# wahn/rs_pbrt

Hardware: NVIDIA H100
Metric: Mrays/s (higher is better)
Workload: dtype f32

## Files before the change

rs_pbrt_b200/csrc/pb_kernels.cuh:

```cuda
#pragma once
#include "pb_bsdf.cuh"
#include "pb_interaction.cuh"
#include "pb_sobol.cuh"
#include "pb_texture.cuh"
#include "pb_material.cuh"

namespace pb {

#define PB_TRACE_THREADS 128
#define PB_TRACE_SMEM_BYTES 49152
#define PB_SHADE_THREADS 128
#define PB_SMEM_SOBOL_BYTES 49152

#ifdef PB_HOST_EMU
PB_D void mbar_init(uint64_t*, uint32_t) {}
PB_D void mbar_fence_init() {}
PB_D void mbar_expect_tx(uint64_t*, uint32_t) {}
PB_D void tma_bulk_g2s(void* dst_smem, const void* src_gmem, uint32_t bytes, uint64_t*) { memcpy(dst_smem, src_gmem, bytes); }
PB_D void mbar_wait(uint64_t*, uint32_t) { __syncthreads(); }
#define PB_DYNAMIC_SMEM(name) unsigned char* name = emu::g_dyn_smem
#else
#define PB_DYNAMIC_SMEM(name) extern __shared__ __align__(16) unsigned char name[]
PB_D void mbar_fence_init() { asm volatile("fence.mbarrier_init.release.cluster;" ::: "memory"); }
PB_D uint32_t smem_u32(const void* p) { return (uint32_t)__cvta_generic_to_shared(p); }
// ... 288 lines not shown
            const float* p0 = vp + 3 * (size_t)(m.vbase + v0);
            const float* p1 = vp + 3 * (size_t)(m.vbase + v1);
            const float* p2 = vp + 3 * (size_t)(m.vbase + v2);
            tv[3 * (size_t)i] = make_float4(p0[0], p0[1], p0[2], p1[0]);
            tv[3 * (size_t)i + 1] = make_float4(p1[1], p1[2], p2[0], p2[1]);
            tv[3 * (size_t)i + 2] = make_float4(p2[2], __uint_as_float(material), __uint_as_float((uint32_t)area_light), __uint_as_float(m.flags));
            tidx[i] = make_uint4(m.vbase + v0, m.vbase + v1, m.vbase + v2, mesh);
        }
    }
    if (err) atomicMax(status, err);
}

__global__ void __launch_bounds__(256) k_wide_build(const float4* __restrict__ nodes, uint32_t n_nodes, float4* __restrict__ wide) {
    const uint32_t i = blockIdx.x * blockDim.x + threadIdx.x;
    if (i >= n_nodes) return;
    const float4 m1 = nodes[2 * (size_t)i + 1];
    const uint32_t meta = __float_as_uint(m1.w);
    if (meta & 0xffffu) return;
    const uint32_t c[2] = {i + 1u, __float_as_uint(m1.z)};
    float4 a[2], b[2];
    uint32_t ref[2];
    for (int k = 0; k < 2; ++k) {
        a[k] = nodes[2 * (size_t)c[k]];
        b[k] = nodes[2 * (size_t)c[k] + 1];
        const uint32_t cm = __float_as_uint(b[k].w), np = cm & 0xffffu;
        ref[k] = np ? (__float_as_uint(b[k].z) | (np << PB_WIDE_LEAF_SHIFT)) : c[k];
    }
    float4* o = wide + 4 * (size_t)i;
    o[0] = make_float4(a[0].x, a[0].y, a[0].z, a[0].w);
    o[1] = make_float4(b[0].x, b[0].y, a[1].x, a[1].y);
    o[2] = make_float4(a[1].z, a[1].w, b[1].x, b[1].y);
    o[3] = make_float4(__uint_as_float(ref[0]), __uint_as_float(ref[1]), __uint_as_float((meta >> 16) & 3u), 0.0f);
}
#ifndef PB_WIDE_MIN_BLOCKS
#define PB_WIDE_MIN_BLOCKS 0
#endif
#ifndef PB_WIDE_INST_MIN_BLOCKS
#define PB_WIDE_INST_MIN_BLOCKS 8
#endif
#if PB_WIDE_MIN_BLOCKS > 0
#define PB_WIDE_BOUNDS __launch_bounds__(PB_TRACE_THREADS, PB_WIDE_MIN_BLOCKS)
#else
#define PB_WIDE_BOUNDS __launch_bounds__(PB_TRACE_THREADS)
#endif
__global__ void PB_WIDE_BOUNDS k_trace_wide_plain(DScene sc, TraceIO io, const uint32_t* __restrict__ d_nrays, uint32_t* __restrict__ cursor, DCounters* cnt, int walk_steps) {
    trace_rays_wide<false>(sc, sc.wide, sc.tri_verts, io, *d_nrays, cursor, cnt, walk_steps);
}
__global__ void __launch_bounds__(PB_TRACE_THREADS, PB_WIDE_INST_MIN_BLOCKS) k_trace_wide_inst(DScene sc, TraceIO io, const uint32_t* __restrict__ d_nrays, uint32_t* __restrict__ cursor,
                                                                                             DCounters* cnt, int walk_steps) {
    trace_rays_wide<true>(sc, sc.wide, sc.tri_verts, io, *d_nrays, cursor, cnt, walk_steps);
}

__global__ void PB_WIDE_BOUNDS k_trace_wide_spec(DScene sc, TraceIO io, const uint32_t* __restrict__ d_nrays,
                                                                                        uint32_t* __restrict__ cursor, DCounters* cnt, int walk_steps) {
    trace_rays_wide_spec(sc, sc.wide, sc.tri_verts, io, *d_nrays, cursor, cnt, walk_steps);
}

__global__ void __launch_bounds__(256) k_rayprep(const float4* __restrict__ rays, const uint32_t* __restrict__ d_nrays, float4* __restrict__ pre) {
    const uint32_t n = *d_nrays;
    for (uint32_t i = blockIdx.x * blockDim.x + threadIdx.x; i < n; i += gridDim.x * blockDim.x) {
        const float4 a = rays[2 * (size_t)i], b = rays[2 * (size_t)i + 1];
        const RayPre r = make_ray(mk3(a.x, a.y, a.z), mk3(b.x, b.y, b.z));
        float4 p0, p1;
        pack_ray(r, p0, p1);
        pre[2 * (size_t)i] = p0;
        pre[2 * (size_t)i + 1] = p1;
    }
}

__global__ void __launch_bounds__(256) k_sort(DScene sc, DPaths ps, DLightGrid grid, uint32_t spatial, uint32_t instancing, const uint32_t* __restrict__ queue,
                                             const uint32_t* __restrict__ d_count, uint32_t* __restrict__ cls_queue, uint32_t cls_stride,
                                             uint32_t* __restrict__ cls_count, uint32_t* __restrict__ reset_count_out, uint32_t* __restrict__ reset_nrays) {
    if (blockIdx.x == 0 && threadIdx.x == 0) { *reset_count_out = 0u; *reset_nrays = 0u; }
    const uint32_t count = *d_count;
    const uint32_t lane = threadIdx.x & 31;
    const uint32_t total = (count + 31u) & ~31u;
    for (uint32_t qi = blockIdx.x * blockDim.x + threadIdx.x; qi < total; qi += gridDim.x * blockDim.x) {
        uint32_t cls = 0xffffffffu, slot = 0;
        if (qi < count) {
// ... 754 lines not shown
```

rs_pbrt_b200/csrc/pb_scene.cuh:

```cuda
#pragma once
#include "pb_math.cuh"

namespace pb {

enum LobeKind { LOBE_SPEC_REFL = 0, LOBE_SPEC_TRANS, LOBE_FRESNEL_SPEC, LOBE_LAMBERT, LOBE_OREN_NAYAR, LOBE_MF_REFL, LOBE_MF_TRANS, LOBE_FRESNEL_BLEND,
                LOBE_LAMBERT_TRANS  };
enum { BSDF_REFLECTION = 1, BSDF_TRANSMISSION = 2, BSDF_DIFFUSE = 4, BSDF_GLOSSY = 8, BSDF_SPECULAR = 16, BSDF_ALL = 31 };
enum FresnelKind { FRESNEL_NOOP = 0, FRESNEL_CONDUCTOR, FRESNEL_DIELECTRIC };

struct DLobe {
    int kind, type, fresnel;
    int has_sc;
    float r[3];
    float t[3];
    float eta_a, eta_b;
    float fr_a[3];
    float fr_k[3];
    float alpha_x, alpha_y;
    float on_a, on_b;
};
PB_HD float* lobe_sc_slot(DLobe& l) {
    if (l.kind == LOBE_FRESNEL_SPEC || l.kind == LOBE_FRESNEL_BLEND) return l.fr_k;
    return (l.kind == LOBE_SPEC_TRANS || l.kind == LOBE_LAMBERT_TRANS || l.kind == LOBE_MF_TRANS) ? l.r : l.t;
}
// ... 44 lines not shown
    float max_anisotropy;
    float su, sv, du, dv;
    uint32_t off[PB_MAX_MIP_LEVELS];
    uint32_t mapping;
    float map_m[16];
    uint32_t kind;
    float value[3];
    uint32_t child[3];
};
struct DMatSrc {
    uint32_t kind;
    float params[24];
    uint32_t tex[8];
    float alpha_u, alpha_v;
    uint8_t tex_off[8];
    uint32_t n_spectrum;
    uint32_t bump;
};
#define PB_MAT_BUMPED 0x200
#define PB_MAT_TEXTURED 0x100

enum { TRI_FLIP = 1, TRI_HAS_N = 2, TRI_HAS_UV = 4, TRI_HAS_S = 8, TRI_INSTANCE = 16 ,
       TRI_ALPHA = 32, TRI_SHADOW_ALPHA = 64  };

struct DInstance {
    uint32_t root, identity, pad0, pad1;
    float m[16], m_inv[16];
};

struct DScene {
    const float4* nodes;
    uint32_t n_nodes;
    const float4* wide;
    const float4* tri_verts;
    uint32_t n_tris;
    const uint4* tri_idx;
    const float* vn;
    const float* vuv;
    const float* vs;
    const DMaterial* materials;
    uint32_t n_materials;
    const DLight* lights;
    float world_radius;
    uint32_t n_lights;
    const DEnv* envs;
    const DInstance* instances;
    uint32_t n_instances;
    const uint2* mesh_alpha;
    const DTexture* textures;
    const DMatSrc* mat_src;
    const float* ewa_lut;
    uint32_t n_textures;
    float dx_camera[3], dy_camera[3];
    uint32_t n_inf;
    uint32_t inf[4];
    float raster_to_camera[16], camera_to_world[16];
    float lens_radius, focal_distance, shutter_open, shutter_close;
    float wb_min[3], wb_max[3];
};

struct DLightGrid {
    int nv[3];
    int n_lights;
    int* state;
    float* func;
    float* cdf;
// ... 79 lines not shown
```

rs_pbrt_b200/csrc/pb_trace.cuh:

```cuda
#pragma once
#include "pb_scene.cuh"

namespace pb {

struct RayPre {
    V3 o, d;
    V3 inv_dir;
    int neg[3];
    uint32_t negmask;
    int kx, ky, kz;
    float sx, sy, sz;
};

PB_D RayPre make_ray(V3 o, V3 d) {
    RayPre r;
    r.o = o;
    r.d = d;
    r.inv_dir = mk3(1.0f / d.x, 1.0f / d.y, 1.0f / d.z);
    r.neg[0] = r.inv_dir.x < 0.0f;
    r.neg[1] = r.inv_dir.y < 0.0f;
    r.neg[2] = r.inv_dir.z < 0.0f;
    r.negmask = (uint32_t)r.neg[0] | ((uint32_t)r.neg[1] << 1) | ((uint32_t)r.neg[2] << 2);
    r.kz = maxdim(abs3(d));
    r.kx = r.kz + 1; if (r.kx == 3) r.kx = 0;
// ... 115 lines not shown
PB_D void load_tri(const float4* __restrict__ tv, uint32_t i, V3& p0, V3& p1, V3& p2) {
    float4 a = __ldg(tv + 3 * (size_t)i), b = __ldg(tv + 3 * (size_t)i + 1), c = __ldg(tv + 3 * (size_t)i + 2);
    p0 = mk3(a.x, a.y, a.z);
    p1 = mk3(a.w, b.x, b.y);
    p2 = mk3(b.z, b.w, c.x);
}

struct WorkCount { uint32_t nodes, tris; };

#ifndef PB_SMEM_STACK_ENTRIES
#define PB_SMEM_STACK_ENTRIES 24
#endif
#define PB_TRACE_THREADS_ 128
#ifndef PB_LEAF_MIN
#define PB_LEAF_MIN 1
#endif
#ifndef PB_FLAT_WALK
#define PB_FLAT_WALK 1
#endif
#ifndef PB_REFILL_MIN
#define PB_REFILL_MIN 1
#endif
#ifndef PB_WALK_STEPS
#define PB_WALK_STEPS 16
#endif

#ifndef PB_CACHE_HINTS
#define PB_CACHE_HINTS 1
#endif
PB_D float4 ldg4_keep(const float4* p) {
#if PB_CACHE_HINTS
    float4 v;
    asm volatile("ld.global.nc.L1::evict_last.v4.f32 {%0,%1,%2,%3}, [%4];" : "=f"(v.x), "=f"(v.y), "=f"(v.z), "=f"(v.w) : "l"(p));
    return v;
#else
    return __ldg(p);
#endif
}
PB_D float4 ldg4_stream(const float4* p) {
#if PB_CACHE_HINTS
    float4 v;
    asm volatile("ld.global.nc.L1::no_allocate.v4.f32 {%0,%1,%2,%3}, [%4];" : "=f"(v.x), "=f"(v.y), "=f"(v.z), "=f"(v.w) : "l"(p));
    return v;
#else
    return __ldg(p);
#endif
}
PB_D float4 lds4(const float4* p) {
#ifdef PB_HOST_EMU
    return *p;
#else
    float4 v;
    asm volatile("ld.shared.v4.f32 {%0,%1,%2,%3}, [%4];" : "=f"(v.x), "=f"(v.y), "=f"(v.z), "=f"(v.w) : "r"((uint32_t)__cvta_generic_to_shared(p)));
    return v;
#endif
}

PB_D void xf_ray_dev(const float* __restrict__ m, V3 o, V3 d, float& t_max, V3& o_out, V3& d_out) {
    const float x = o.x, y = o.y, z = o.z;
    V3 ow = mk3(m[0] * x + m[1] * y + m[2] * z + m[3], m[4] * x + m[5] * y + m[6] * z + m[7], m[8] * x + m[9] * y + m[10] * z + m[11]);
    const float wp = m[12] * x + m[13] * y + m[14] * z + m[15];
    const V3 o_err = mk3(fabsf(m[0] * x) + fabsf(m[1] * y) + fabsf(m[2] * z) + fabsf(m[3]), fabsf(m[4] * x) + fabsf(m[5] * y) + fabsf(m[6] * z) + fabsf(m[7]),
                         fabsf(m[8] * x) + fabsf(m[9] * y) + fabsf(m[10] * z) + fabsf(m[11])) * gamma_n(3);
    if (wp != 1.0f) { const float inv = 1.0f / wp; ow = mk3(inv * ow.x, inv * ow.y, inv * ow.z); }
    const V3 dw = mk3(m[0] * d.x + m[1] * d.y + m[2] * d.z, m[4] * d.x + m[5] * d.y + m[6] * d.z, m[8] * d.x + m[9] * d.y + m[10] * d.z);
    const float ls = len2(dw);
// ... 444 lines not shown
            }
            if (!entered) {
                leaf_n = 0;
                if (!done) {
                    uint32_t nxt = 0;
                    PB_WPOP();
                    PB_WGOTO();
                }
            }
        }
        if (active && done) {
            if (INST && !any_hit && !hit_flag) best_prim = -1;
            const uint32_t slot = dest & PB_RAY_SLOT_MASK, kind = dest >> 30;
            if (kind == RAY_SHADOW) io.occl[slot] = best_prim >= 0 ? 1u : 0u;
            else {
                const float4 rec = make_float4(__int_as_float(best_prim), best.b0, best.b1, best.b2);
                if (kind == RAY_EXTEND) { io.hit[slot] = rec; if (INST) io.hit_inst[slot] = (uint32_t)best_inst; }
                else { io.mis_hit[slot] = rec; if (INST) io.mis_inst[slot] = (uint32_t)best_inst; }
            }
            active = false;
        }
    }
#undef PB_WPOP
#undef PB_WGOTO
#undef PB_WPUSH
    uint32_t a = n_closest, b = n_shadow;
    for (int o = 16; o > 0; o >>= 1) { a += __shfl_xor_sync(FULL, a, o); b += __shfl_xor_sync(FULL, b, o); }
    if (lane == 0) {
        if (a) atomicAdd(&cnt->closest_rays, (unsigned long long)a);
        if (b) atomicAdd(&cnt->shadow_rays, (unsigned long long)b);
    }
}

PB_D void trace_rays_wide_spec(const DScene& sc, const float4* __restrict__ wide, const float4* __restrict__ tris, const TraceIO& io, uint32_t n_rays,
                               uint32_t* __restrict__ cursor, DCounters* cnt, int walk_steps) {
    const unsigned FULL = 0xffffffffu;
    const int lane = threadIdx.x & 31;
    constexpr int NS = PB_WIDE_STACK_ENTRIES;
    __shared__ uint32_t s_ref[NS][PB_TRACE_THREADS_];
    __shared__ float s_tmin[NS][PB_TRACE_THREADS_];
    uint32_t l_ref[64 - NS];
    float l_tmin[64 - NS];
    RayPre r;
    float t_max = 0.0f, cur_tmin = 0.0f, leaf2_tmin = 0.0f;
    THit best;
    int best_prim = -1;
    uint32_t sp = 0, cur = 0, dest = 0, leaf1 = 0, leaf2 = 0;
    bool active = false, any_hit = false, exhausted = n_rays == 0, have_cur = false;
    uint32_t n_closest = 0, n_shadow = 0;
    const float neg_inf = __int_as_float((int)0xff800000);
#define PB_SPOP()                                                                                               \
    do {                                                                                                        \
        found = false;                                                                                          \
        while (sp != 0u) {                                                                                      \
            --sp;                                                                                               \
            const uint32_t e_ = sp < (uint32_t)NS ? s_ref[sp][threadIdx.x] : l_ref[sp - NS];                    \
            const float m_ = sp < (uint32_t)NS ? s_tmin[sp][threadIdx.x] : l_tmin[sp - NS];                     \
            if (m_ < t_max) { nxt = e_; tm = m_; found = true; break; }                                         \
        }                                                                                                       \
    } while (0)
#define PB_SROUTE()                                                                                             \
    do {                                                                                                        \
        for (;;) {                                                                                              \
            if (!found) { have_cur = false; break; }                                                            \
            if (!(nxt >> PB_WIDE_LEAF_SHIFT)) { cur = nxt; cur_tmin = tm; have_cur = true; break; }             \
            if (!leaf1) { leaf1 = nxt; PB_SPOP(); continue; }                                                   \
// ... 105 lines not shown
```

rs_pbrt_b200/csrc/pbrt_gpu.cu:

```cuda
#include <sched.h>

#include <algorithm>
#include <chrono>
#include <cmath>
#include <cstdio>
#include <cstdlib>
#include <atomic>
#include <cstring>
#include <functional>
#include <map>
#include <memory>
#include <mutex>
#include <string>
#include <thread>
#include <vector>

#include "../../include/pbrt_gpu.h"
#include "pb_kernels.cuh"
#include "pb_direct.cuh"

using namespace pb;

extern "C" {
extern const unsigned char pb_sobol_blob_start[];
// ... 423 lines not shown
    std::vector<cudaEvent_t> ev_pool;
    size_t ev_used = 0;
    cudaError_t event(cudaEvent_t* e) {
        if (ev_used == ev_pool.size()) {
            cudaEvent_t n;
            cudaError_t rc = cudaEventCreate(&n);
            if (rc != cudaSuccess) return rc;
            ev_pool.push_back(n);
        }
        *e = ev_pool[ev_used++];
        return cudaSuccess;
    }
    std::mutex mu;
};
static size_t lightgrid_budget() {
    if (const char* e = std::getenv("PB_LIGHTGRID_BYTES")) {
        const long long v = std::atoll(e);
        if (v > 0) return (size_t)v;
    }
    return (size_t)4 << 30;
}
static DeviceScratch* scratch_for(int device) {
    static DeviceScratch* pool[64] = {nullptr};
    static std::mutex pool_mu;
    std::lock_guard<std::mutex> g(pool_mu);
    if (device < 0 || device >= 64) return nullptr;
    if (!pool[device]) pool[device] = new DeviceScratch();
    return pool[device];
}

struct PbrtScene {
    int device = 0;
    DScene d;
    DevBuf<float4> nodes, tri_verts, wide;
    DevBuf<uint4> tri_idx;
    DevBuf<float> vn, vuv, vs;
    DevBuf<DMaterial> materials, materials_single;
    DevBuf<DLight> lights;
    DevBuf<uint32_t> m32, nib;
    DevBuf<uint64_t> vdc, vdci;
    DevBuf<float> halton;
    std::vector<DLight> h_lights;
    std::vector<uint32_t> h_nib;
    struct EnvBufs { DevBuf<float4> texels; DevBuf<float> cond_func, cond_cdf, cond_int, marg_func, marg_cdf; };
    std::vector<std::unique_ptr<EnvBufs>> env_bufs;
    DevBuf<DEnv> envs;
    DevBuf<DInstance> instances;
    DevBuf<uint2> mesh_alpha;
    std::vector<std::unique_ptr<DevBuf<float4>>> tex_bufs;
    DevBuf<DTexture> textures;
    DevBuf<DMatSrc> mat_src;
    DevBuf<float> ewa_lut;
    std::vector<Sp> h_env_power;
    bool has_null_material = false;
    bool area_only = true;
    uint32_t class_mask = 0;
    size_t upload_bytes = 0;
    DevBuf<DCounters> counters;
    DevBuf<float> film, samples;
    size_t capacity = 0;
    void recycle_buffers(int dev) {
        nodes.cache_dev = tri_verts.cache_dev = wide.cache_dev = tri_idx.cache_dev = vn.cache_dev = vuv.cache_dev = vs.cache_dev = dev;
        materials.cache_dev = materials_single.cache_dev = lights.cache_dev = m32.cache_dev = nib.cache_dev = vdc.cache_dev = vdci.cache_dev = halton.cache_dev = dev;
        envs.cache_dev = instances.cache_dev = mesh_alpha.cache_dev = textures.cache_dev = mat_src.cache_dev = ewa_lut.cache_dev = counters.cache_dev = dev;
    }
};

static bool wide_enabled() {
    static const bool on = !(getenv("PB_WIDE") && atoi(getenv("PB_WIDE")) == 0);
    return on;
}
static bool wide_spec_enabled() {
    static const bool on = getenv("PB_WIDE_SPEC") && atoi(getenv("PB_WIDE_SPEC")) != 0;
    return on;
}
struct TraceLauncher {
    bool count_work = false, inst = false, smem = false, alpha = false, wide = false, wide_spec = false;
    int wide_walk = 16;
    size_t smem_bytes = 0;
    int grid = 1, blocks_per_sm = 1;
    template <typename F> void with_kernel(F&& f) const {
        if (alpha) {
            if (inst) { if (count_work) f(k_trace<true, 0, false, true, true>); else f(k_trace<false, 0, false, true, true>); }
            else { if (count_work) f(k_trace<true, 0, false, false, true>); else f(k_trace<false, 0, false, false, true>); }
        } else if (inst) { if (count_work) f(k_trace<true, 0, false, true>); else f(k_trace<false, 0, false, true>); }
        else if (smem) { if (count_work) f(k_trace<true, 0, true>); else f(k_trace<false, 0, true>); }
        else { if (count_work) f(k_trace<true, 0, false>); else f(k_trace<false, 0, false>); }
    }
    cudaError_t init(const PbrtScene* sc, bool count, int sm_count) {
        count_work = count;
        inst = sc->d.n_instances > 0;
        alpha = sc->d.mesh_alpha != nullptr;
        const size_t scene_bytes = (size_t)sc->d.n_nodes * 32 + (size_t)sc->d.n_tris * 48;
        smem = !inst && !alpha && scene_bytes > 0 && scene_bytes <= PB_TRACE_SMEM_BYTES;
        smem_bytes = smem ? scene_bytes : 0;
        wide = wide_enabled() && sc->d.wide != nullptr && !count_work && !alpha && !smem;
        {
            int l2 = 0;
            cudaDeviceGetAttribute(&l2, cudaDevAttrL2CacheSize, sc->device);
            wide_walk = (size_t)sc->d.n_nodes * 64 > (size_t)std::max(l2, 1) ? 6 : 16;
            if (const char* e_ = getenv("PB_WIDE_WALK")) wide_walk = std::min(64, std::max(1, atoi(e_)));
        }
        int bps = 1;
        cudaError_t e = cudaSuccess;
        wide_spec = wide && !inst && wide_spec_enabled();
        if (wide_spec) e = cudaOccupancyMaxActiveBlocksPerMultiprocessor(&bps, k_trace_wide_spec, PB_TRACE_THREADS, 0);
        else if (wide) e = inst ? cudaOccupancyMaxActiveBlocksPerMultiprocessor(&bps, k_trace_wide_inst, PB_TRACE_THREADS, 0)
                           : cudaOccupancyMaxActiveBlocksPerMultiprocessor(&bps, k_trace_wide_plain, PB_TRACE_THREADS, 0);
        else with_kernel([&](auto k) { e = cudaOccupancyMaxActiveBlocksPerMultiprocessor(&bps, k, PB_TRACE_THREADS, smem_bytes); });
        blocks_per_sm = bps;
        grid = sm_count * std::max(1, bps);
        return e;
    }
    void launch(const DScene& d, const TraceIO& io, const uint32_t* d_nrays, uint32_t* d_cursor, DCounters* cnt, cudaStream_t s) const {
        if (wide_spec) k_trace_wide_spec<<<grid, PB_TRACE_THREADS, 0, s>>>(d, io, d_nrays, d_cursor, cnt, wide_walk);
        else if (wide) {
            if (inst) k_trace_wide_inst<<<grid, PB_TRACE_THREADS, 0, s>>>(d, io, d_nrays, d_cursor, cnt, wide_walk);
            else k_trace_wide_plain<<<grid, PB_TRACE_THREADS, 0, s>>>(d, io, d_nrays, d_cursor, cnt, wide_walk);
        } else if (alpha) {
            if (inst) { if (count_work) k_trace<true, 0, false, true, true><<<grid, PB_TRACE_THREADS, 0, s>>>(d, io, d_nrays, 0, d_cursor, cnt); else k_trace<false, 0, false, true, true><<<grid, PB_TRACE_THREADS, 0, s>>>(d, io, d_nrays, 0, d_cursor, cnt); }
            else { if (count_work) k_trace<true, 0, false, false, true><<<grid, PB_TRACE_THREADS, 0, s>>>(d, io, d_nrays, 0, d_cursor, cnt); else k_trace<false, 0, false, false, true><<<grid, PB_TRACE_THREADS, 0, s>>>(d, io, d_nrays, 0, d_cursor, cnt); }
        } else if (inst) {
            if (count_work) k_trace<true, 0, false, true><<<grid, PB_TRACE_THREADS, 0, s>>>(d, io, d_nrays, 0, d_cursor, cnt);
            else k_trace<false, 0, false, true><<<grid, PB_TRACE_THREADS, 0, s>>>(d, io, d_nrays, 0, d_cursor, cnt);
        } else if (smem) {
            if (count_work) k_trace<true, 0, true><<<grid, PB_TRACE_THREADS, smem_bytes, s>>>(d, io, d_nrays, 0, d_cursor, cnt);
            else k_trace<false, 0, true><<<grid, PB_TRACE_THREADS, smem_bytes, s>>>(d, io, d_nrays, 0, d_cursor, cnt);
        } else {
            if (count_work) k_trace<true, 0, false><<<grid, PB_TRACE_THREADS, 0, s>>>(d, io, d_nrays, 0, d_cursor, cnt);
            else k_trace<false, 0, false><<<grid, PB_TRACE_THREADS, 0, s>>>(d, io, d_nrays, 0, d_cursor, cnt);
        }
    }
};

static unsigned host_threads() {
    static const unsigned n = [] {
        unsigned c = std::max(1u, std::thread::hardware_concurrency());
        cpu_set_t set;
        if (sched_getaffinity(0, sizeof set, &set) == 0) c = std::max(1, CPU_COUNT(&set));
        if (FILE* f = fopen("/sys/fs/cgroup/cpu.max", "r")) {
            char quota[32] = {0};
            long period = 0;
            if (fscanf(f, "%31s %ld", quota, &period) == 2 && strcmp(quota, "max") != 0 && period > 0) c = std::min<unsigned>(c, (unsigned)std::max(1L, (atol(quota) + period / 2) / period));
            fclose(f);
        }
        if (const char* w = getenv("LOCAL_WORLD_SIZE")) c = std::max(1u, c / (unsigned)std::max(1, atoi(w)));
        return std::min(32u, c);
    }();
// ... 456 lines not shown
    std::memcpy(vdc.data(), blob + 32 + m32.size() * 4, vdc.size() * 8);
    std::memcpy(vdci.data(), blob + 32 + m32.size() * 4 + vdc.size() * 8, vdci.size() * 8);
    std::vector<uint32_t> nib((size_t)1024 * PB_SOBOL_CHUNKS * 16);
    for (int dim = 0; dim < 1024; ++dim)
        for (int c = 0; c < PB_SOBOL_CHUNKS; ++c)
            for (int e = 0; e < 16; ++e) {
                uint32_t v = 0;
                for (int j = 0; j < 4; ++j)
                    if (e & (1 << j)) v ^= m32[(size_t)dim * 52 + 4 * c + j];
                nib[((size_t)dim * PB_SOBOL_CHUNKS + c) * 16 + e] = v;
            }
    std::vector<float> halton(128 * 5);
    for (int s = 0; s < 128; ++s)
        for (int k = 0; k < 5; ++k) halton[5 * s + k] = host_radical_inverse(k, (uint64_t)s);

    since("tables built");
    sc->has_null_material = has_null;
    sc->h_nib = nib;
    for (const DLight& l : lights) if (l.kind != PBRT_LIGHT_DIFFUSE_AREA) sc->area_only = false;
    for (const DMaterial& m : mats) sc->class_mask |= 1u << (m.cls & 0xff);
    sc->h_lights = lights;
#define UP(buf, vec)                                                                                     \
    do {                                                                                                 \
        cudaError_t e_ = sc->buf.upload(vec);                                                            \
        if (e_ != cudaSuccess) return fail(PBRT_E_CUDA, std::string("upload " #buf ": ") + cudaGetErrorString(e_)); \
        sc->upload_bytes += (vec).size() * sizeof((vec)[0]);                                             \
    } while (0)
    sc->upload_bytes += up_bytes;
    since("nodes + triangles uploaded");
    {
        bool ok = desc->n_nodes > 1 && desc->nodes[0].n_prims == 0 && !any_alpha &&
                  desc->n_nodes < (1u << PB_WIDE_LEAF_SHIFT) && desc->n_tris < (1u << PB_WIDE_LEAF_SHIFT) &&
                  (desc->n_instances > 0 || (size_t)desc->n_nodes * 32 + (size_t)desc->n_tris * 48 > PB_TRACE_SMEM_BYTES) && max_leaf_prims.load() <= 15u;
        if (ok) {
            CK(sc->wide.alloc(4 * (size_t)desc->n_nodes));
            k_wide_build<<<(desc->n_nodes + 255) / 256, 256>>>(sc->nodes.p, desc->n_nodes, sc->wide.p);
            CK(cudaGetLastError());
            g_launches++;
        }
    }
    {
        std::vector<DEnv> envs;
        sc->h_env_power.assign(desc->n_lights, sp1(0.0f));
        for (uint32_t k = 0; k < n_inf; ++k) {
            const PbrtLight& l = desc->lights[inf_idx[k]];
            HostEnv he;
            build_env(l.env_texels, (int)l.env_res[0], (int)l.env_res[1], he);
            sc->env_bufs.emplace_back(new PbrtScene::EnvBufs());
            PbrtScene::EnvBufs& b = *sc->env_bufs.back();
            cudaError_t e_ = b.texels.upload(he.texels);
            if (e_ == cudaSuccess) e_ = b.cond_func.upload(he.cond_func);
            if (e_ == cudaSuccess) e_ = b.cond_cdf.upload(he.cond_cdf);
            if (e_ == cudaSuccess) e_ = b.cond_int.upload(he.cond_int);
            if (e_ == cudaSuccess) e_ = b.marg_func.upload(he.marg_func);
            if (e_ == cudaSuccess) e_ = b.marg_cdf.upload(he.marg_cdf);
            if (e_ != cudaSuccess) { return fail(PBRT_E_CUDA, std::string("upload environment map: ") + cudaGetErrorString(e_)); }
            sc->upload_bytes += he.texels.size() * 16 + (he.cond_func.size() + he.cond_cdf.size() + he.cond_int.size() + he.marg_func.size() + he.marg_cdf.size()) * 4;
            DEnv de;
            std::memset(&de, 0, sizeof de);
            de.texels = b.texels.p; de.w = he.w; de.h = he.h; de.nu = he.nu; de.nv = he.nv;
            de.cond_func = b.cond_func.p; de.cond_cdf = b.cond_cdf.p; de.cond_int = b.cond_int.p;
            de.marg_func = b.marg_func.p; de.marg_cdf = b.marg_cdf.p; de.marg_int = he.marg_int;
            std::memcpy(de.l2w, l.l2w, sizeof de.l2w);
            std::memcpy(de.w2l, l.w2l, sizeof de.w2l);
            lights[inf_idx[k]].env = (uint32_t)envs.size();
            envs.push_back(de);
            sc->h_env_power[inf_idx[k]] = he.power_L;
// ... 33 lines not shown
            DTexture& dt = dtex[i];
            std::memset(&dt, 0, sizeof dt);
            std::vector<float4> flat;
            for (size_t l = 0; l < pyr.size(); ++l) {
                dt.off[l] = (uint32_t)flat.size();
                for (const Sp& v : pyr[l].t) flat.push_back(make_float4(v.r, v.g, v.b, 0.0f));
            }
            sc->tex_bufs.emplace_back(new DevBuf<float4>());
            cudaError_t e_ = sc->tex_bufs.back()->upload(flat);
            if (e_ != cudaSuccess) { return fail(PBRT_E_CUDA, std::string("upload texture: ") + cudaGetErrorString(e_)); }
            sc->upload_bytes += flat.size() * 16;
            dt.texels = sc->tex_bufs.back()->p;
            dt.w = pyr[0].us; dt.h = pyr[0].vs; dt.n_levels = (int)pyr.size();
            dt.wrap = t.wrap; dt.trilinear = t.trilinear ? 1u : 0u; dt.max_anisotropy = t.max_anisotropy;
            dt.su = t.su; dt.sv = t.sv; dt.du = t.du; dt.dv = t.dv;
            dt.mapping = t.mapping;
            std::memcpy(dt.map_m, t.map_m, sizeof dt.map_m);
        }
        std::vector<float> lut(128);
        for (int i = 0; i < 128; ++i) {
            const float alpha = 2.0f, r2 = (float)i / (float)(128 - 1);
            lut[i] = expf(-alpha * r2) - expf(-alpha);
        }
        UP(textures, dtex); UP(mat_src, mat_src); UP(ewa_lut, lut);
    }
    for (uint32_t i = 0; i < desc->n_materials; ++i) mats_single[i].cls = mats[i].cls;
    UP(materials_single, mats_single);
    UP(materials, mats); UP(lights, lights); UP(m32, m32); UP(nib, nib); UP(vdc, vdc); UP(vdci, vdci); UP(halton, halton);
#undef UP
    DScene& d = sc->d;
    std::memset(&d, 0, sizeof d);
    d.nodes = sc->nodes.p; d.n_nodes = desc->n_nodes;
    d.wide = sc->wide.p;
    d.tri_verts = sc->tri_verts.p; d.n_tris = desc->n_tris;
    d.tri_idx = sc->tri_idx.p;
    d.vn = sc->vn.p; d.vuv = sc->vuv.p; d.vs = sc->vs.p;
    d.materials = sc->materials.p; d.n_materials = desc->n_materials;
    d.lights = sc->lights.p; d.n_lights = desc->n_lights;
    d.envs = sc->envs.p; d.n_inf = n_inf;
    d.instances = sc->instances.p; d.n_instances = desc->n_instances;
    d.mesh_alpha = sc->mesh_alpha.p;
    d.textures = sc->textures.p; d.mat_src = sc->mat_src.p; d.ewa_lut = sc->ewa_lut.p; d.n_textures = desc->n_textures;
    {
        auto r2c = [&](float x, float y) {
            const float* m = desc->camera.raster_to_camera;
            V3 r = mk3(m[0] * x + m[1] * y + m[2] * 0.0f + m[3], m[4] * x + m[5] * y + m[6] * 0.0f + m[7], m[8] * x + m[9] * y + m[10] * 0.0f + m[11]);
            const float w = m[12] * x + m[13] * y + m[14] * 0.0f + m[15];
            if (w != 1.0f) { const float inv = 1.0f / w; r = mk3(inv * r.x, inv * r.y, inv * r.z); }
            return r;
        };
        const V3 r0 = r2c(0.0f, 0.0f), dx = r2c(1.0f, 0.0f) - r0, dy = r2c(0.0f, 1.0f) - r0;
        d.dx_camera[0] = dx.x; d.dx_camera[1] = dx.y; d.dx_camera[2] = dx.z;
        d.dy_camera[0] = dy.x; d.dy_camera[1] = dy.y; d.dy_camera[2] = dy.z;
    }
    for (uint32_t k = 0; k < n_inf; ++k) d.inf[k] = inf_idx[k];
    std::memcpy(d.raster_to_camera, desc->camera.raster_to_camera, 64);
    std::memcpy(d.camera_to_world, desc->camera.camera_to_world, 64);
    d.lens_radius = desc->camera.lens_radius; d.focal_distance = desc->camera.focal_distance;
    d.shutter_open = desc->camera.shutter_open; d.shutter_close = desc->camera.shutter_close;
    for (int k = 0; k < 3; ++k) { d.wb_min[k] = desc->world_bound[k]; d.wb_max[k] = desc->world_bound[3 + k]; }
    {
        V3 pmin = mk3(d.wb_min[0], d.wb_min[1], d.wb_min[2]), pmax = mk3(d.wb_max[0], d.wb_max[1], d.wb_max[2]);
        V3 c = vdiv(pmin + pmax, 2.0f);
        bool inside = c.x >= pmin.x && c.x <= pmax.x && c.y >= pmin.y && c.y <= pmax.y && c.z >= pmin.z && c.z <= pmax.z;
        d.world_radius = inside ? len3(c - pmax) : 0.0f;
    }
// ... 1128 lines not shown
```

Baseline: 1503.

## Add 4-wide BVH layout and traversal kernel for scenes exceeding L2

Adds a 4-wide BVH built by collapsing each binary node with its grandchildren into a 128-byte record, plus a traversal kernel that tests four boxes per step and orders children by ray direction. It is used by default only for non-instanced scenes whose binary wide BVH would not fit in L2, and it gets its own walk-step defaults. The aim is fewer dependent node fetches and traversal steps per ray, at the cost of larger records, more registers and extra stack handling.

```diff
diff --git a/rs_pbrt_b200/csrc/pb_kernels.cuh b/rs_pbrt_b200/csrc/pb_kernels.cuh
--- a/rs_pbrt_b200/csrc/pb_kernels.cuh
+++ b/rs_pbrt_b200/csrc/pb_kernels.cuh
@@ -344,8 +344,61 @@
     o[2] = make_float4(a[1].z, a[1].w, b[1].x, b[1].y);
     o[3] = make_float4(__uint_as_float(ref[0]), __uint_as_float(ref[1]), __uint_as_float((meta >> 16) & 3u), 0.0f);
 }
+PB_D bool box_in_box(const float4 a, const float4 b, const float4 pa, const float4 pb) {
+    const float big = 3.402823466e38f;
+    return fabsf(pa.x) <= big && fabsf(pa.y) <= big && fabsf(pa.z) <= big && fabsf(pa.w) <= big && fabsf(pb.x) <= big && fabsf(pb.y) <= big &&
+           fabsf(a.x) <= big && fabsf(a.y) <= big && fabsf(a.z) <= big && fabsf(a.w) <= big && fabsf(b.x) <= big && fabsf(b.y) <= big &&
+           pa.x <= a.x && pa.y <= a.y && pa.z <= a.z && a.w <= pa.w && b.x <= pb.x && b.y <= pb.y;
+}
+__global__ void __launch_bounds__(256) k_wide4_build(const float4* __restrict__ nodes, uint32_t n_nodes, float4* __restrict__ wide4) {
+    const uint32_t i = blockIdx.x * blockDim.x + threadIdx.x;
+    if (i >= n_nodes) return;
+    const float4 m1 = nodes[2 * (size_t)i + 1];
+    const uint32_t meta = __float_as_uint(m1.w);
+    if (meta & 0xffffu) return;
+    const float nan = __int_as_float(0x7fc00000);
+    float box[24];
+    uint32_t ref[4], axes = (meta >> 16) & 3u;
+    for (int s = 0; s < 24; ++s) box[s] = nan;
+    for (int s = 0; s < 4; ++s) ref[s] = 0u;
+    auto put = [&](int s, uint32_t node, const float4 a, const float4 b) {
+        const uint32_t np = __float_as_uint(b.w) & 0xffffu;
+        ref[s] = np ? (__float_as_uint(b.z) | (np << PB_WIDE_LEAF_SHIFT)) : node;
+        box[6 * s] = a.x; box[6 * s + 1] = a.y; box[6 * s + 2] = a.z; box[6 * s + 3] = a.w; box[6 * s + 4] = b.x; box[6 * s + 5] = b.y;
+    };
+    const uint32_t c[2] = {i + 1u, __float_as_uint(m1.z)};
+    for (int k = 0; k < 2; ++k) {
+        const float4 a = nodes[2 * (size_t)c[k]], b = nodes[2 * (size_t)c[k] + 1];
+        const uint32_t cm = __float_as_uint(b.w);
+        bool expand = (cm & 0xffffu) == 0u;
+        float4 ga[2], gb[2];
+        const uint32_t g[2] = {c[k] + 1u, __float_as_uint(b.z)};
+        if (expand) {
+            for (int j = 0; j < 2; ++j) {
+                ga[j] = nodes[2 * (size_t)g[j]];
+                gb[j] = nodes[2 * (size_t)g[j] + 1];
+                expand = expand && box_in_box(ga[j], gb[j], a, b);
+            }
+        }
+        if (expand) {
+            put(2 * k, g[0], ga[0], gb[0]);
+            put(2 * k + 1, g[1], ga[1], gb[1]);
+            axes |= ((cm >> 16) & 3u) << (2 + 2 * k);
+        } else put(2 * k, c[k], a, b);
+    }
+    float4* o = wide4 + 8 * (size_t)i;
+    for (int q = 0; q < 6; ++q) o[q] = make_float4(box[4 * q], box[4 * q + 1], box[4 * q + 2], box[4 * q + 3]);
+    o[6] = make_float4(__uint_as_float(ref[0]), __uint_as_float(ref[1]), __uint_as_float(ref[2]), __uint_as_float(ref[3]));
+    o[7] = make_float4(__uint_as_float(axes), 0.0f, 0.0f, 0.0f);
+}
 #ifndef PB_WIDE_MIN_BLOCKS
 #define PB_WIDE_MIN_BLOCKS 0
+#endif
+#ifndef PB_WIDE4_WALK_BIG
+#define PB_WIDE4_WALK_BIG 4
+#endif
+#ifndef PB_WIDE4_WALK_SMALL
+#define PB_WIDE4_WALK_SMALL 8
 #endif
 #ifndef PB_WIDE_INST_MIN_BLOCKS
 #define PB_WIDE_INST_MIN_BLOCKS 8
@@ -357,6 +410,9 @@
 #endif
 __global__ void PB_WIDE_BOUNDS k_trace_wide_plain(DScene sc, TraceIO io, const uint32_t* __restrict__ d_nrays, uint32_t* __restrict__ cursor, DCounters* cnt, int walk_steps) {
     trace_rays_wide<false>(sc, sc.wide, sc.tri_verts, io, *d_nrays, cursor, cnt, walk_steps);
+}
+__global__ void PB_WIDE_BOUNDS k_trace_wide4_plain(DScene sc, TraceIO io, const uint32_t* __restrict__ d_nrays, uint32_t* __restrict__ cursor, DCounters* cnt, int walk_steps) {
+    trace_rays_wide4(sc, sc.wide4, sc.tri_verts, io, *d_nrays, cursor, cnt, walk_steps);
 }
 __global__ void __launch_bounds__(PB_TRACE_THREADS, PB_WIDE_INST_MIN_BLOCKS) k_trace_wide_inst(DScene sc, TraceIO io, const uint32_t* __restrict__ d_nrays, uint32_t* __restrict__ cursor,
                                                                                              DCounters* cnt, int walk_steps) {
diff --git a/rs_pbrt_b200/csrc/pb_scene.cuh b/rs_pbrt_b200/csrc/pb_scene.cuh
--- a/rs_pbrt_b200/csrc/pb_scene.cuh
+++ b/rs_pbrt_b200/csrc/pb_scene.cuh
@@ -100,6 +100,7 @@
     const float4* nodes;
     uint32_t n_nodes;
     const float4* wide;
+    const float4* wide4;
     const float4* tri_verts;
     uint32_t n_tris;
     const uint4* tri_idx;
diff --git a/rs_pbrt_b200/csrc/pb_trace.cuh b/rs_pbrt_b200/csrc/pb_trace.cuh
--- a/rs_pbrt_b200/csrc/pb_trace.cuh
+++ b/rs_pbrt_b200/csrc/pb_trace.cuh
@@ -171,6 +171,15 @@
 #if PB_CACHE_HINTS
     float4 v;
     asm volatile("ld.global.nc.L1::evict_last.v4.f32 {%0,%1,%2,%3}, [%4];" : "=f"(v.x), "=f"(v.y), "=f"(v.z), "=f"(v.w) : "l"(p));
+    return v;
+#else
+    return __ldg(p);
+#endif
+}
+PB_D uint32_t ldg1_keep(const uint32_t* p) {
+#if PB_CACHE_HINTS
+    uint32_t v;
+    asm volatile("ld.global.nc.L1::evict_last.u32 %0, [%1];" : "=r"(v) : "l"(p));
     return v;
 #else
     return __ldg(p);
@@ -681,6 +690,139 @@
     }
 }
 
+#define PB_WIDE4_STACK 128
+PB_D void trace_rays_wide4(const DScene& sc, const float4* __restrict__ wide4, const float4* __restrict__ tris, const TraceIO& io, uint32_t n_rays,
+                           uint32_t* __restrict__ cursor, DCounters* cnt, int walk_steps) {
+    const unsigned FULL = 0xffffffffu;
+    const int lane = threadIdx.x & 31;
+    constexpr int NS = PB_WIDE_STACK_ENTRIES;
+    __shared__ uint32_t s_ref[NS][PB_TRACE_THREADS_];
+    __shared__ float s_tmin[NS][PB_TRACE_THREADS_];
+    uint32_t l_ref[PB_WIDE4_STACK - NS];
+    float l_tmin[PB_WIDE4_STACK - NS];
+    RayPre r;
+    float t_max = 0.0f;
+    THit best;
+    int best_prim = -1;
+    uint32_t sp = 0, cur = 0, dest = 0, leaf_off = 0, leaf_n = 0;
+    bool active = false, any_hit = false, exhausted = n_rays == 0;
+    uint32_t n_closest = 0, n_shadow = 0;
+#define PB_W4PUSH(ref_, tmin_)                                                                                  \
+    do {                                                                                                        \
+        if (sp < (uint32_t)NS) { s_ref[sp][threadIdx.x] = (ref_); s_tmin[sp][threadIdx.x] = (tmin_); }           \
+        else { l_ref[sp - NS] = (ref_); l_tmin[sp - NS] = (tmin_); }                                            \
+        ++sp;                                                                                                   \
+    } while (0)
+#define PB_W4POP()                                                                                              \
+    do {                                                                                                        \
+        for (;;) {                                                                                              \
+            if (sp == 0u) { done = true; break; }                                                               \
+            --sp;                                                                                               \
+            const uint32_t e_ = sp < (uint32_t)NS ? s_ref[sp][threadIdx.x] : l_ref[sp - NS];                    \
+            const float m_ = sp < (uint32_t)NS ? s_tmin[sp][threadIdx.x] : l_tmin[sp - NS];                     \
+            if (m_ < t_max) { nxt = e_; break; }                                                                \
+        }                                                                                                       \
+    } while (0)
+#define PB_W4GOTO()                                                                                             \
+    do {                                                                                                        \
+        if (!done) {                                                                                            \
+            if (nxt >> PB_WIDE_LEAF_SHIFT) { leaf_n = nxt >> PB_WIDE_LEAF_SHIFT; leaf_off = nxt & ((1u << PB_WIDE_LEAF_SHIFT) - 1u); } \
+            else cur = nxt;                                                                                     \
+        }                                                                                                       \
+    } while (0)
+#define PB_W4SWAP(c_, a_, b_) do { if (c_) { const auto s_ = (a_); (a_) = (b_); (b_) = s_; } } while (0)
+    for (;;) {
+        unsigned idle = __ballot_sync(FULL, !active);
+        bool done = false;
+        if (idle && !exhausted) {
+            uint32_t base = 0;
+            if (lane == 0) base = atomicAdd(cursor, (uint32_t)__popc(idle));
+            base = __shfl_sync(FULL, base, 0);
+            if (base >= n_rays) exhausted = true;
+            const uint32_t my = base + (uint32_t)__popc(idle & ((1u << lane) - 1u));
+            if (!active && my < n_rays) {
+                const uint32_t qi = io.perm ? __ldg(io.perm + my) : my;
+                const float4 a = ldg4_stream(io.rays + 2 * (size_t)qi), b = ldg4_stream(io.rays + 2 * (size_t)qi + 1);
+                t_max = a.w;
+                dest = __float_as_uint(b.w);
+                any_hit = (dest >> 30) == RAY_SHADOW;
+                r = make_ray(mk3(a.x, a.y, a.z), mk3(b.x, b.y, b.z));
+                best_prim = -1;
+                best.t = 0.0f; best.b0 = best.b1 = best.b2 = 0.0f;
+                sp = 0; cur = 0; leaf_n = 0;
+                active = true;
+                if (any_hit) n_shadow++; else n_closest++;
+                const float4 n0 = ldg4_keep(sc.nodes), n1 = ldg4_keep(sc.nodes + 1);
+                done = !slab_test(n0, n1, r, t_max);
+            }
+        }
+        if (!__any_sync(FULL, active)) break;
+        for (int step = 0; step < walk_steps; ++step) {
+            if (!(active && !done && leaf_n == 0u)) break;
+            const float4* rec = wide4 + 8 * (size_t)cur;
+            const float4 f0 = ldg4_keep(rec), f1 = ldg4_keep(rec + 1), f2 = ldg4_keep(rec + 2), f3 = ldg4_keep(rec + 3);
+            const float4 f4 = ldg4_keep(rec + 4), f5 = ldg4_keep(rec + 5), f6 = ldg4_keep(rec + 6);
+            const uint32_t axes = ldg1_keep(reinterpret_cast<const uint32_t*>(rec + 7));
+            float t0, t1, t2, t3;
+            bool h0 = slab_geo(f0.x, f0.y, f0.z, f0.w, f1.x, f1.y, r, t0) && t0 < t_max;
+            bool h1 = slab_geo(f1.z, f1.w, f2.x, f2.y, f2.z, f2.w, r, t1) && t1 < t_max;
+            bool h2 = slab_geo(f3.x, f3.y, f3.z, f3.w, f4.x, f4.y, r, t2) && t2 < t_max;
+            bool h3 = slab_geo(f4.z, f4.w, f5.x, f5.y, f5.z, f5.w, r, t3) && t3 < t_max;
+            uint32_t r0 = __float_as_uint(f6.x), r1 = __float_as_uint(f6.y), r2 = __float_as_uint(f6.z), r3 = __float_as_uint(f6.w);
+            const bool neg_c0 = ((r.negmask >> ((axes >> 2) & 3u)) & 1u) != 0u, neg_c1 = ((r.negmask >> ((axes >> 4) & 3u)) & 1u) != 0u;
+            const bool neg_n = ((r.negmask >> (axes & 3u)) & 1u) != 0u;
+            PB_W4SWAP(neg_c0, h0, h1); PB_W4SWAP(neg_c0, t0, t1); PB_W4SWAP(neg_c0, r0, r1);
+            PB_W4SWAP(neg_c1, h2, h3); PB_W4SWAP(neg_c1, t2, t3); PB_W4SWAP(neg_c1, r2, r3);
+            PB_W4SWAP(neg_n, h0, h2); PB_W4SWAP(neg_n, t0, t2); PB_W4SWAP(neg_n, r0, r2);
+            PB_W4SWAP(neg_n, h1, h3); PB_W4SWAP(neg_n, t1, t3); PB_W4SWAP(neg_n, r1, r3);
+            if (h3 && (h0 || h1 || h2)) PB_W4PUSH(r3, t3);
+            if (h2 && (h0 || h1)) PB_W4PUSH(r2, t2);
+            if (h1 && h0) PB_W4PUSH(r1, t1);
+            uint32_t nxt = h0 ? r0 : (h1 ? r1 : (h2 ? r2 : r3));
+            if (!(h0 || h1 || h2 || h3)) PB_W4POP();
+            PB_W4GOTO();
+        }
+        if (active && leaf_n) {
+            for (uint32_t i = 0; i < leaf_n; ++i) {
+                const float4* tp = tris + 3 * (size_t)(leaf_off + i);
+                const float4 a = ldg4_stream(tp), b = ldg4_stream(tp + 1), c = ldg4_stream(tp + 2);
+                THit h;
+                if (tri_test(mk3(a.x, a.y, a.z), mk3(a.w, b.x, b.y), mk3(b.z, b.w, c.x), r, t_max, h)) {
+                    t_max = h.t;
+                    best = h;
+                    best_prim = (int)(leaf_off + i);
+                    if (any_hit) { done = true; break; }
+                }
+            }
+            leaf_n = 0;
+            if (!done) {
+                uint32_t nxt = 0;
+                PB_W4POP();
+                PB_W4GOTO();
+            }
+        }
+        if (active && done) {
+            const uint32_t slot = dest & PB_RAY_SLOT_MASK, kind = dest >> 30;
+            if (kind == RAY_SHADOW) io.occl[slot] = best_prim >= 0 ? 1u : 0u;
+            else {
+                const float4 rec = make_float4(__int_as_float(best_prim), best.b0, best.b1, best.b2);
+                if (kind == RAY_EXTEND) io.hit[slot] = rec; else io.mis_hit[slot] = rec;
+            }
+            active = false;
+        }
+    }
+#undef PB_W4SWAP
+#undef PB_W4GOTO
+#undef PB_W4POP
+#undef PB_W4PUSH
+    uint32_t a = n_closest, b = n_shadow;
+    for (int o = 16; o > 0; o >>= 1) { a += __shfl_xor_sync(FULL, a, o); b += __shfl_xor_sync(FULL, b, o); }
+    if (lane == 0) {
+        if (a) atomicAdd(&cnt->closest_rays, (unsigned long long)a);
+        if (b) atomicAdd(&cnt->shadow_rays, (unsigned long long)b);
+    }
+}
+
 PB_D void trace_rays_wide_spec(const DScene& sc, const float4* __restrict__ wide, const float4* __restrict__ tris, const TraceIO& io, uint32_t n_rays,
                                uint32_t* __restrict__ cursor, DCounters* cnt, int walk_steps) {
     const unsigned FULL = 0xffffffffu;
diff --git a/rs_pbrt_b200/csrc/pbrt_gpu.cu b/rs_pbrt_b200/csrc/pbrt_gpu.cu
--- a/rs_pbrt_b200/csrc/pbrt_gpu.cu
+++ b/rs_pbrt_b200/csrc/pbrt_gpu.cu
@@ -479,7 +479,7 @@
 struct PbrtScene {
     int device = 0;
     DScene d;
-    DevBuf<float4> nodes, tri_verts, wide;
+    DevBuf<float4> nodes, tri_verts, wide, wide4;
     DevBuf<uint4> tri_idx;
     DevBuf<float> vn, vuv, vs;
     DevBuf<DMaterial> materials, materials_single;
@@ -507,7 +507,7 @@
     DevBuf<float> film, samples;
     size_t capacity = 0;
     void recycle_buffers(int dev) {
-        nodes.cache_dev = tri_verts.cache_dev = wide.cache_dev = tri_idx.cache_dev = vn.cache_dev = vuv.cache_dev = vs.cache_dev = dev;
+        nodes.cache_dev = tri_verts.cache_dev = wide.cache_dev = wide4.cache_dev = tri_idx.cache_dev = vn.cache_dev = vuv.cache_dev = vs.cache_dev = dev;
         materials.cache_dev = materials_single.cache_dev = lights.cache_dev = m32.cache_dev = nib.cache_dev = vdc.cache_dev = vdci.cache_dev = halton.cache_dev = dev;
         envs.cache_dev = instances.cache_dev = mesh_alpha.cache_dev = textures.cache_dev = mat_src.cache_dev = ewa_lut.cache_dev = counters.cache_dev = dev;
     }
@@ -517,12 +517,21 @@
     static const bool on = !(getenv("PB_WIDE") && atoi(getenv("PB_WIDE")) == 0);
     return on;
 }
+static bool wide_beyond_l2(uint32_t n_nodes, int device) {
+    int l2 = 0;
+    cudaDeviceGetAttribute(&l2, cudaDevAttrL2CacheSize, device);
+    return (size_t)n_nodes * 64 > (size_t)std::max(l2, 1);
+}
+static bool wide4_wanted(uint32_t n_nodes, int device) {
+    static const int mode = getenv("PB_WIDE4") ? (atoi(getenv("PB_WIDE4")) != 0 ? 1 : 0) : -1;
+    return mode < 0 ? wide_beyond_l2(n_nodes, device) : mode == 1;
+}
 static bool wide_spec_enabled() {
     static const bool on = getenv("PB_WIDE_SPEC") && atoi(getenv("PB_WIDE_SPEC")) != 0;
     return on;
 }
 struct TraceLauncher {
-    bool count_work = false, inst = false, smem = false, alpha = false, wide = false, wide_spec = false;
+    bool count_work = false, inst = false, smem = false, alpha = false, wide = false, wide4 = false, wide_spec = false;
     int wide_walk = 16;
     size_t smem_bytes = 0;
     int grid = 1, blocks_per_sm = 1;
@@ -541,17 +550,18 @@
         const size_t scene_bytes = (size_t)sc->d.n_nodes * 32 + (size_t)sc->d.n_tris * 48;
         smem = !inst && !alpha && scene_bytes > 0 && scene_bytes <= PB_TRACE_SMEM_BYTES;
         smem_bytes = smem ? scene_bytes : 0;
-        wide = wide_enabled() && sc->d.wide != nullptr && !count_work && !alpha && !smem;
+        wide = wide_enabled() && (sc->d.wide != nullptr || sc->d.wide4 != nullptr) && !count_work && !alpha && !smem;
+        wide4 = wide && sc->d.wide4 != nullptr;
         {
-            int l2 = 0;
-            cudaDeviceGetAttribute(&l2, cudaDevAttrL2CacheSize, sc->device);
-            wide_walk = (size_t)sc->d.n_nodes * 64 > (size_t)std::max(l2, 1) ? 6 : 16;
+            const bool big = wide_beyond_l2(sc->d.n_nodes, sc->device);
+            wide_walk = wide4 ? (big ? PB_WIDE4_WALK_BIG : PB_WIDE4_WALK_SMALL) : (big ? 6 : 16);
             if (const char* e_ = getenv("PB_WIDE_WALK")) wide_walk = std::min(64, std::max(1, atoi(e_)));
         }
         int bps = 1;
         cudaError_t e = cudaSuccess;
         wide_spec = wide && !inst && wide_spec_enabled();
         if (wide_spec) e = cudaOccupancyMaxActiveBlocksPerMultiprocessor(&bps, k_trace_wide_spec, PB_TRACE_THREADS, 0);
+        else if (wide4) e = cudaOccupancyMaxActiveBlocksPerMultiprocessor(&bps, k_trace_wide4_plain, PB_TRACE_THREADS, 0);
         else if (wide) e = inst ? cudaOccupancyMaxActiveBlocksPerMultiprocessor(&bps, k_trace_wide_inst, PB_TRACE_THREADS, 0)
                            : cudaOccupancyMaxActiveBlocksPerMultiprocessor(&bps, k_trace_wide_plain, PB_TRACE_THREADS, 0);
         else with_kernel([&](auto k) { e = cudaOccupancyMaxActiveBlocksPerMultiprocessor(&bps, k, PB_TRACE_THREADS, smem_bytes); });
@@ -561,6 +571,7 @@
     }
     void launch(const DScene& d, const TraceIO& io, const uint32_t* d_nrays, uint32_t* d_cursor, DCounters* cnt, cudaStream_t s) const {
         if (wide_spec) k_trace_wide_spec<<<grid, PB_TRACE_THREADS, 0, s>>>(d, io, d_nrays, d_cursor, cnt, wide_walk);
+        else if (wide4) k_trace_wide4_plain<<<grid, PB_TRACE_THREADS, 0, s>>>(d, io, d_nrays, d_cursor, cnt, wide_walk);
         else if (wide) {
             if (inst) k_trace_wide_inst<<<grid, PB_TRACE_THREADS, 0, s>>>(d, io, d_nrays, d_cursor, cnt, wide_walk);
             else k_trace_wide_plain<<<grid, PB_TRACE_THREADS, 0, s>>>(d, io, d_nrays, d_cursor, cnt, wide_walk);
@@ -1083,7 +1094,12 @@
         bool ok = desc->n_nodes > 1 && desc->nodes[0].n_prims == 0 && !any_alpha &&
                   desc->n_nodes < (1u << PB_WIDE_LEAF_SHIFT) && desc->n_tris < (1u << PB_WIDE_LEAF_SHIFT) &&
                   (desc->n_instances > 0 || (size_t)desc->n_nodes * 32 + (size_t)desc->n_tris * 48 > PB_TRACE_SMEM_BYTES) && max_leaf_prims.load() <= 15u;
-        if (ok) {
+        if (ok && desc->n_instances == 0 && wide4_wanted(desc->n_nodes, device) && !wide_spec_enabled()) {
+            CK(sc->wide4.alloc(8 * (size_t)desc->n_nodes));
+            k_wide4_build<<<(desc->n_nodes + 255) / 256, 256>>>(sc->nodes.p, desc->n_nodes, sc->wide4.p);
+            CK(cudaGetLastError());
+            g_launches++;
+        } else if (ok) {
             CK(sc->wide.alloc(4 * (size_t)desc->n_nodes));
             k_wide_build<<<(desc->n_nodes + 255) / 256, 256>>>(sc->nodes.p, desc->n_nodes, sc->wide.p);
             CK(cudaGetLastError());
@@ -1183,6 +1199,7 @@
     std::memset(&d, 0, sizeof d);
     d.nodes = sc->nodes.p; d.n_nodes = desc->n_nodes;
     d.wide = sc->wide.p;
+    d.wide4 = sc->wide4.p;
     d.tri_verts = sc->tri_verts.p; d.n_tris = desc->n_tris;
     d.tri_idx = sc->tri_idx.p;
     d.vn = sc->vn.p; d.vuv = sc->vuv.p; d.vs = sc->vs.p;
```

After: 1544, median of 6. 2.8% higher.
